# evoldoers/machineboss

Measured on NVIDIA B200. Metric: forward_viterbi_gcups, higher is better.
Workload: dtype f64

## Files before the change

machineboss_b200/csrc/mb_jit.cu:

```cuda
#include <cuda.h>
#include <dlfcn.h>
#include <nvrtc.h>
#include <unistd.h>

#include <algorithm>
#include <cmath>
#include <cstdio>
#include <cstring>
#include <map>
#include <mutex>
#include <sstream>

#include "mb_internal.h"
#include "mb_jit_skeleton.h"

namespace mb {

struct Driver {
  CUresult (*ModuleLoadData) (CUmodule*, const void*) = nullptr;
  CUresult (*ModuleUnload) (CUmodule) = nullptr;
  CUresult (*ModuleGetFunction) (CUfunction*, CUmodule, const char*) = nullptr;
  CUresult (*ModuleGetGlobal) (CUdeviceptr*, size_t*, CUmodule, const char*) = nullptr;
  CUresult (*LaunchKernel) (CUfunction, unsigned, unsigned, unsigned, unsigned, unsigned, unsigned, unsigned, CUstream, void**, void**) = nullptr;
  CUresult (*FuncSetAttribute) (CUfunction, CUfunction_attribute, int) = nullptr;
// ... 893 lines not shown
    o << "#ifndef MB_LDS\n"
         "template<int OFF> __device__ __forceinline__ double mb_lds (const unsigned addr) { double v; asm (\"ld.shared.f64 %0, [%1+%2];\" : \"=d\"(v) : \"r\"(addr), \"n\"(OFF)); return v; }\n"
         "#define MB_LDS(addr, off) mb_lds<off> (addr)\n#endif\n";
    o << "#define MB_PKW " << (passC * J.tbBytes + 3) / 4 << "      // 32-bit words of packed back-pointers per lane and step\n";
    o << "#ifndef MB_HOST_HARNESS\n"
         "// n = max (n, t) with the reference's tie-break (a later candidate wins only if strictly greater); with PTR the\n"
         "// winner's field value replaces the field in `word`: (word & ~field) | val, or a plain OR for a one-bit field\n"
         "template<bool PTR> __device__ __forceinline__ void mb_vmax (double& n, const double t, unsigned& word, const unsigned field, const unsigned val) {\n"
         "  if (!PTR) { if (n < t) n = t; return; }\n"
         "  if (field == val) asm (\"{ .reg .pred p; setp.lt.f64 p, %0, %2; selp.f64 %0, %2, %0, p; @p or.b32 %1, %1, %3; }\" : \"+d\"(n), \"+r\"(word) : \"d\"(t), \"r\"(val));\n"
         "  else asm (\"{ .reg .pred p; setp.lt.f64 p, %0, %2; selp.f64 %0, %2, %0, p; @p lop3.b32 %1, %1, %3, %4, 0xEA; }\" : \"+d\"(n), \"+r\"(word) : \"d\"(t), \"r\"(~field), \"r\"(val));\n"
         "}\n#endif\n\n";
    gen_cell_row_vit (o, m, J.fwd, J);
    gen_cell_row_lin (o, m, J.fwd, true);
    gen_cell_row_lin (o, m, J.bwd, false);
    o << "// MB_ROWCELLS_END\n";
  }
  gen_cell (o, m, J.fwd, true, false, J);
  gen_cell (o, m, J.bwd, false, false, J);
  gen_cell (o, m, J.fwd, true, true, J);
  gen_cell_counts (o, m, J);
  gen_cell_lin (o, m, J.fwd, true);
  gen_cell_lin (o, m, J.bwd, false);
  gen_cell_counts_lin (o, m, J);
  gen_fstore_lin (o, m, J);
  o << kJitSkeleton;
  return o.str();
}

int jit_host_tables (const mb_machine* m, int which, std::vector<double>& out) {
  std::string why;
  if (!jit_supported (m, &why)) { set_error ("machine not eligible for the JIT engine: " + why); return 1; }
  JitEngine J;
  generate (m, J);
  std::vector<double> ef, eb;
  fill_weights (m, J, ef, eb);
  RowTables f, b;
  row_tables (m, J.fwd, true, f);
  row_tables (m, J.bwd, false, b);
  const int nf = std::max (J.fwd.nSil, 1), nb = std::max (J.bwd.nSil, 1);
  out.clear();
  if (which == 0) out = f.rowLog;
  else if (which == 1) out = f.rowLinN;
  else if (which == 2) out = b.rowLinN;
  else if (which == 3) { const double* sp = (const double*) J.silParam.data(); out.assign (sp, sp + nf + nb); }
  else if (which == 4) {
    out.insert (out.end(), f.silN.begin(), f.silN.begin() + nf);
    out.insert (out.end(), b.silN.begin(), b.silN.begin() + nb);
    out.push_back (f.originInv); out.push_back (b.originInv); out.push_back (f.resLog); out.push_back (b.resLog);
  } else if (which == 5) out.push_back (f.ok && b.ok && J.linearOK ? 1. : 0.);
  else { set_error ("mb_jit_host_tables: which must be 0..5"); return 1; }
  return 0;
}

int jit_compile_check (const mb_machine* m, std::string* log) {
  std::string why;
  if (!jit_supported (m, &why)) { set_error ("machine not eligible for the JIT engine: " + why); return 1; }
  JitEngine J;
  generate (m, J);
  std::vector<char> cubin;
  if (nvrtc_compile (J.source, "", cubin, log)) return 1;
  if (!J.sourceV.empty()) {
    std::string logV;
    if (nvrtc_compile (J.sourceV, ".viterbi.cu", cubin, &logV)) return 1;
    if (log) *log += "\n---- Viterbi module (MB_C = " + std::to_string (J.CV) + ") ----\n" + logV;
  }
  if (m->opt.get ("jit_split", -1) > 0) {
    std::string logS;
    if (nvrtc_compile (J.sourceS, ".split.cu", cubin, &logS)) return 1;
    if (log) *log += "\n---- split-mode module ----\n" + logS;
  }
  return 0;
}

int jit_prepare (mb_machine* m) {
  JitEngine* Jp = new JitEngine;
  m->jit = Jp;
  JitEngine& J = *Jp;
  generate (m, J);
  if (compile (m, J)) return 1;

  std::vector<double> ef, eb;
  fill_weights (m, J, ef, eb);
  MB_CUDA (cudaMalloc (&J.dEmitF, ef.size() * 8));
  MB_CUDA (cudaMalloc (&J.dEmitB, eb.size() * 8));
  MB_CUDA (cudaMalloc (&J.dEmitFLin, ef.size() * 8));
  MB_CUDA (cudaMalloc (&J.dEmitBLin, eb.size() * 8));
  MB_CUDA (cudaMalloc (&J.dCounter, 8));
  if (jit_update_weights (m)) return 1;
  MB_CUDA (cudaMalloc (&J.dIdTabB, std::max<size_t> (J.bwd.idTab.size(), 1) * 4));
  MB_CUDA (cudaMemcpy (J.dIdTabB, J.bwd.idTab.data(), J.bwd.idTab.size() * 4, cudaMemcpyHostToDevice));
  std::vector<int32_t> plan;
  for (int v: J.fwd.stateSlot0) plan.push_back (v);
  for (auto& s: J.fwd.slots) plan.push_back (s.type);
  for (auto& s: J.fwd.slots) plan.push_back (s.other);
  for (auto& s: J.fwd.slots) plan.push_back (s.idOff);
  for (int v: J.shift) plan.push_back (v);
  for (int v: J.bits) plan.push_back (v);
  for (int v: J.fwd.idTab) plan.push_back (v);
  MB_CUDA (cudaMalloc (&J.dTbPlan, std::max<size_t> (plan.size(), 1) * 4));
  MB_CUDA (cudaMemcpy (J.dTbPlan, plan.data(), plan.size() * 4, cudaMemcpyHostToDevice));
  return 0;
}

void jit_destroy (mb_machine* m) {
  if (!m->jit) return;
  JitEngine* J = (JitEngine*) m->jit;
  if (J->mod && g_drv.ModuleUnload) g_drv.ModuleUnload (J->mod);
  if (J->modV && g_drv.ModuleUnload) g_drv.ModuleUnload (J->modV);
  if (J->modS && g_drv.ModuleUnload) g_drv.ModuleUnload (J->modS);
  for (auto& f: J->fit) if (f.mod && g_drv.ModuleUnload) g_drv.ModuleUnload (f.mod);
  if (J->dEmitF) cudaFree (J->dEmitF);
  if (J->dEmitB) cudaFree (J->dEmitB);
  if (J->dEmitFLin) cudaFree (J->dEmitFLin);
  if (J->dEmitBLin) cudaFree (J->dEmitBLin);
  if (J->dTbPlan) cudaFree (J->dTbPlan);
  if (J->dIdTabB) cudaFree (J->dIdTabB);
  if (J->dCounter) cudaFree (J->dCounter);
  if (J->dRowVit) cudaFree (J->dRowVit);
  if (J->dRowFLinN) cudaFree (J->dRowFLinN);
  if (J->dRowBLinN) cudaFree (J->dRowBLinN);
  delete J;
  m->jit = nullptr;
}

struct MBArgsHost {
  const uint8_t* x; const int64_t* xOff;
  const uint8_t* y; const int64_t* yOff;
  const int64_t* order; int64_t nWork; unsigned long long* counter;
  double* bnd; int64_t bndStride;
  double* result;
  const double* emit;
  uint8_t* tb; const int64_t* tbOff;
  double* F; const int64_t* fOff;
  const double* ll;
  double* counts;
  const int32_t* idTabB;
  int32_t* flag;
  unsigned* F32; const int64_t* f32Off;
  int32_t* ef; const int64_t* efOff;
  const int64_t* items; const int64_t* itemBnd; int* prog;
};

struct DevBuf {
  void* p = nullptr;
  ~DevBuf() { if (p) cudaFree (p); }
  int alloc (size_t bytes) { MB_CUDA (cudaMalloc (&p, bytes ? bytes : 8)); return 0; }
  template<class T> T* as() { return (T*) p; }
};

static std::vector<int64_t> cost_order (const mb_batch* b, const std::vector<int64_t>& pairs) {
  std::vector<int64_t> o = pairs;
  std::stable_sort (o.begin(), o.end(), [&] (int64_t p, int64_t q) {
    const double cp = (double) (b->xOff[p + 1] - b->xOff[p] + 1) * (double) (b->yOff[p + 1] - b->yOff[p] + 1);
    const double cq = (double) (b->xOff[q + 1] - b->xOff[q] + 1) * (double) (b->yOff[q + 1] - b->yOff[q] + 1);
    return cp > cq;
  });
  return o;
}

static const std::vector<int64_t>& full_order (mb_batch* b) {
  if ((int64_t) b->fullOrder.size() != b->nPairs) {
    std::vector<int64_t> all ((size_t) b->nPairs);
    for (int64_t k = 0; k < b->nPairs; ++k) all[k] = k;
    b->fullOrder = cost_order (b, all);
    b->wsOrderHoldsFull = false;
  }
  return b->fullOrder;
}

struct CountArgs { double* F = nullptr; const int64_t* fOff = nullptr; const double* ll = nullptr; double* counts = nullptr; int32_t* flag = nullptr;
                   unsigned* F32 = nullptr; const int64_t* f32Off = nullptr; int32_t* ef = nullptr; const int64_t* efOff = nullptr; };

static int launch (mb_machine* m, mb_batch* b, int which, const std::vector<int64_t>& order, double* dResult, uint8_t* dTb, const int64_t* dTbOff,
                   const CountArgs& ca = CountArgs(), int useC = 0) {
  JitEngine& J = *(JitEngine*) m->jit;
  const bool scoreKernel = which == 2 || which == 5 || which == 6 || which == 9;
  bool narrow = useC == J.C && useC != J.CV;
  const int scoreIdx = which == 2 ? 0 : which == 5 ? 1 : which == 6 ? 2 : 3;
  const JitEngine::FitModule* fitM = nullptr;
  if (scoreKernel && useC && useC != J.C && useC != J.CV) {
    for (auto& f: J.fit) if (f.C == useC) fitM = &f;
    if (!fitM) { set_error ("jit engine: no module fitted to " + std::to_string (useC) + " columns per lane"); return 1; }
  }
  if ((which == 5 || which == 6) && !J.normOK) { set_error ("jit engine: the normalised linear sweep was asked for a machine whose unit weights cannot be divided out"); return 1; }
  narrow = narrow && J.modV && scoreKernel;
  const bool rowTab = scoreKernel;
  const int slot = which;
  CUfunction fn = narrow ? (which == 2 ? J.kViterbiN : which == 5 ? J.kForwardLinN : which == 6 ? J.kBackwardLinN : J.kViterbiScoreN)
    : which == 9 ? J.kViterbiScore : which == 0 ? J.kForward : which == 1 ? J.kBackward : which == 2 ? J.kViterbi : which == 3 ? J.kFStore : which == 4 ? J.kBCounts : which == 5 ? J.kForwardLin : which == 6 ? J.kBackwardLin : which == 7 ? J.kFStoreLin : J.kBCountsLin;
  const bool lin = which >= 5 && which <= 8;
  int64_t maxLo = 0;
  for (int64_t k: order) maxLo = std::max (maxLo, b->yOff[k + 1] - b->yOff[k]);
  const int warpsPerBlock = J.threads / 32;
  int64_t grid = (int64_t) J.numSMs * (fitM ? fitM->blocksPerSM[scoreIdx] : narrow ? J.blocksPerSMN[scoreIdx] : J.blocksPerSM[slot]);
  if (fitM) fn = fitM->k[scoreIdx];
  const int W = 32 * (scoreKernel && J.modV ? J.CV : J.C);
  bool split = false;
  std::vector<int64_t> items, itemBnd;
  if (scoreKernel && !narrow && !fitM && m->opt.get ("jit_split", -1) != 0) {
    int64_t nItems = 0;
    for (int64_t k: order) nItems += (b->xOff[k + 1] - b->xOff[k] + W) / W;
    split = nItems > (int64_t) order.size() && (m->opt.get ("jit_split", -1) > 0 || (double) order.size() < 0.75 * (double) (grid * warpsPerBlock));
    if (split) {
      int64_t at = 0;
      for (int64_t k: order) {
        const int64_t nStrips = (b->xOff[k + 1] - b->xOff[k] + W) / W, Lo = b->yOff[k + 1] - b->yOff[k];
        if (nStrips > 0xffff) { split = false; break; }
        for (int64_t st = 0; st < nStrips; ++st) { items.push_back ((k << 16) | st); itemBnd.push_back (at); at += (Lo + 1) * (m->S + 1); }
      }
      itemBnd.push_back (at);
    }
  }
  if (split) {
    if (ensure_split_module (m, J)) return 1;
    const int q = which == 2 ? 0 : which == 5 ? 1 : which == 6 ? 2 : 3;
    fn = J.kSplit[q];
    grid = (int64_t) J.numSMs * J.blocksPerSMS[q];
  }
  const int64_t nWorkItems = split ? (int64_t) items.size() : (int64_t) order.size();
  grid = std::min<int64_t> (grid, (nWorkItems + warpsPerBlock - 1) / warpsPerBlock);
  grid = std::max<int64_t> (grid, 1);
  const int64_t bndStride = 2 * (maxLo + 1) * (m->S + 1);
  if (ws_bytes (b, WS_ORDER) < order.size() * 8) b->wsOrderHoldsFull = false;
  int64_t* dOrder = (int64_t*) ws_reserve (b, WS_ORDER, order.size() * 8);
  double* dBnd = (double*) ws_reserve (b, WS_BND, (size_t) (split ? itemBnd.back() + bndStride : grid * warpsPerBlock * bndStride) * 8);
  unsigned long long* dCounter = (unsigned long long*) ws_reserve (b, WS_COUNTER, 8);
  if (!dOrder || !dBnd || !dCounter) return 1;
  const bool isFull = &order == &b->fullOrder;
  if (!(isFull && b->wsOrderHoldsFull))
    MB_CUDA (cudaMemcpyAsync (dOrder, order.data(), order.size() * 8, cudaMemcpyHostToDevice, b->stream));
  b->wsOrderHoldsFull = isFull;
  MB_CUDA (cudaMemsetAsync (dCounter, 0, 8, b->stream));
  MBArgsHost A;
  A.x = b->dX; A.xOff = b->dXOff; A.y = b->dY; A.yOff = b->dYOff;
  A.order = dOrder; A.nWork = nWorkItems; A.counter = dCounter;
  A.items = nullptr; A.itemBnd = nullptr; A.prog = nullptr;
  if (split) {
    int64_t* dItems = (int64_t*) ws_reserve (b, WS_ITEMS, items.size() * 8);
    int64_t* dItemBnd = (int64_t*) ws_reserve (b, WS_ITEMBND, itemBnd.size() * 8);
    int* dProg = (int*) ws_reserve (b, WS_PROG, items.size() * 4);
    if (!dItems || !dItemBnd || !dProg) return 1;
    MB_CUDA (cudaMemcpyAsync (dItems, items.data(), items.size() * 8, cudaMemcpyHostToDevice, b->stream));
    MB_CUDA (cudaMemcpyAsync (dItemBnd, itemBnd.data(), itemBnd.size() * 8, cudaMemcpyHostToDevice, b->stream));
    MB_CUDA (cudaMemsetAsync (dProg, 0, items.size() * 4, b->stream));
    if (ca.flag) MB_CUDA (cudaMemsetAsync (ca.flag, 0, (size_t) b->nPairs * 4, b->stream));
    A.items = dItems; A.itemBnd = dItemBnd; A.prog = dProg;
  }
  A.bnd = dBnd; A.bndStride = bndStride;
  A.result = dResult;
  A.emit = (which == 5 || which == 7) ? J.dEmitFLin : (which == 6 || which == 8) ? J.dEmitBLin : (which == 1 || which == 4) ? J.dEmitB : J.dEmitF;
  if (rowTab) A.emit = which == 5 ? J.dRowFLinN : which == 6 ? J.dRowBLinN : J.dRowVit;
  A.flag = ca.flag;
  A.F32 = ca.F32; A.f32Off = ca.f32Off; A.ef = ca.ef; A.efOff = ca.efOff;
  A.tb = dTb; A.tbOff = dTbOff;
  A.F = ca.F; A.fOff = ca.fOff; A.ll = ca.ll; A.counts = ca.counts; A.idTabB = J.dIdTabB;
  if (m->opt.get ("verbose", 0))
    fprintf (stderr, "[mb_jit] kernel %d%s grid %lld x %d threads, %zu B smem, %d CTAs/SM, C=%d, %zu pairs, bnd %.1f MB\n", which, split ? " (split: strips as work items)" : rowTab && lin ? " (normalised)" : "", (long long) grid, J.threads,
             J.smemBytes[which], J.blocksPerSM[slot], fitM ? fitM->C : ((which == 2 || which == 5 || which == 6 || which == 9) && !narrow) ? J.CV : J.C, order.size(), (double) (grid * warpsPerBlock * bndStride) * 8 / 1e6);
  void* params[2] = { (rowTab && lin) ? (void*) J.silParamLinN.data() : lin ? (void*) J.silParamLin.data() : (void*) J.silParam.data(), (void*) &A };
  if (!cu_ok (g_drv.LaunchKernel (fn, (unsigned) grid, 1, 1, (unsigned) J.threads, 1, 1, (unsigned) J.smemBytes[which], (CUstream) b->stream, params, nullptr), "cuLaunchKernel")) return 1;
  return 0;
}

int jit_forward (mb_machine* m, mb_batch* b, double* loglike, bool backward) {
  JitEngine& J = *(JitEngine*) m->jit;
  if (b->nPairs == 0) return 0;
  const std::vector<int64_t>& order = full_order (b);
  double* dRes = (double*) ws_reserve (b, WS_RESULT, (size_t) b->nPairs * 8);
  if (!dRes) return 1;
  if (timing_begin (b)) return 1;
  int64_t launches = 1;
  if (J.linearOK && J.normOK) {
    int32_t* dFlag = (int32_t*) ws_reserve (b, WS_FLAG, (size_t) b->nPairs * 4);
    if (!dFlag) return 1;
    CountArgs ca;
    ca.flag = dFlag;
    if (launch (m, b, backward ? 6 : 5, order, dRes, nullptr, nullptr, ca, choose_width (m, J, b, order, 0))) return 1;
    std::vector<int32_t> flag ((size_t) b->nPairs);
    MB_CUDA (cudaMemcpyAsync (loglike, dRes, (size_t) b->nPairs * 8, cudaMemcpyDeviceToHost, b->stream));
    MB_CUDA (cudaMemcpyAsync (flag.data(), dFlag, (size_t) b->nPairs * 4, cudaMemcpyDeviceToHost, b->stream));
    MB_CUDA (cudaStreamSynchronize (b->stream));
    std::vector<int64_t> redo;
    for (int64_t k = 0; k < b->nPairs; ++k) if (flag[k] || !(loglike[k] > -INFINITY)) redo.push_back (k);
    b->lastRedo = (int64_t) redo.size();
    if (m->opt.get ("verbose", 0) && !redo.empty()) {
      int64_t nf[8] = { 0, 0, 0, 0, 0, 0, 0, 0 };
      for (int64_t k = 0; k < b->nPairs; ++k) ++nf[flag[k] & 7];
      fprintf (stderr, "[mb_jit] linear sweep flagged %lld of %lld pairs; by reason mask (1 spread, 2 neighbour frame, 4 boundary frame) 0..7: %lld %lld %lld %lld %lld %lld %lld %lld\n",
               (long long) redo.size(), (long long) b->nPairs, (long long) nf[0], (long long) nf[1], (long long) nf[2], (long long) nf[3], (long long) nf[4], (long long) nf[5], (long long) nf[6], (long long) nf[7]);
    }
    if (!redo.empty()) {
      if (launch (m, b, backward ? 1 : 0, cost_order (b, redo), dRes, nullptr, nullptr)) return 1;
      ++launches;
    }
  } else { b->lastRedo = 0; if (launch (m, b, backward ? 1 : 0, order, dRes, nullptr, nullptr)) return 1; }
  if (timing_end (b, launches)) return 1;
  MB_CUDA (cudaMemcpy (loglike, dRes, (size_t) b->nPairs * 8, cudaMemcpyDeviceToHost));
  return 0;
}

#define TB_MAXS 64
#define TB_MAXSLOTS 256
__global__ void __launch_bounds__(64) jit_traceback_kernel (TbPlan p, int nSlots, DevBatch b, const int64_t* __restrict__ pairs, int64_t nPairsHere,
                                      const uint8_t* __restrict__ tb, const int64_t* __restrict__ tbOff,
                                      const double* __restrict__ score, int64_t* __restrict__ len,
                                      uint8_t* __restrict__ tmp, const int64_t* __restrict__ tmpOff) {
  __shared__ unsigned perState[TB_MAXS + 1];
  __shared__ unsigned char slotMove[TB_MAXSLOTS], slotOther[TB_MAXSLOTS];
  for (int q = threadIdx.x; q <= p.S; q += blockDim.x)
    perState[q] = (q < p.S ? (unsigned) p.shift[q] | ((unsigned) p.bits[q] << 8) : 0u) | ((unsigned) p.stateSlot0[q] << 16);
  for (int q = threadIdx.x; q < nSlots; q += blockDim.x) {
    const int type = p.slotType[q];
    slotMove[q] = (unsigned char) (((type == T_MATCH || type == T_DELETE) ? 1 : 0) | ((type == T_MATCH || type == T_INSERT) ? 2 : 0));
    slotOther[q] = (unsigned char) p.slotOther[q];
  }
  __syncthreads();
  const int64_t slot = (int64_t) blockIdx.x * blockDim.x + threadIdx.x;
  if (slot >= nPairsHere) return;
  const int64_t k = pairs[slot];
  const int64_t Li = b.xOff[k + 1] - b.xOff[k], Lo = b.yOff[k + 1] - b.yOff[k];
  const uint8_t* base = tb + tbOff[k];
  uint8_t* out = tmp + tmpOff[slot + 1];
  int64_t n = 0;
  if (score[k] > -INFINITY) {
    int64_t i = Li, o = Lo;
    int s = p.S - 1;
    auto fetch = [&] (int64_t ii, int64_t oo) {
      const unsigned ui = (unsigned) ii, strip = ui / (unsigned) p.W, within = ui - strip * (unsigned) p.W, lane = within / (unsigned) p.C;
      const uint8_t* wp = base + ((((int64_t) strip * (Lo + 32) + oo + lane) * 32 + lane) * p.laneBytes + (within - lane * (unsigned) p.C) * p.tbBytes);
      if (within >= 8 && oo >= 8) asm volatile ("prefetch.global.L2 [%0];" :: "l"(wp - ((int64_t) (8 + 8 / p.C) * 32 + 8 / p.C) * p.laneBytes));
      unsigned long long w = 0;
      for (int q = 0; q < p.tbBytes; ++q) w |= (unsigned long long) wp[q] << (8 * q);
      return w;
    };
    unsigned long long word = fetch (i, o);
    while (i > 0 || o > 0 || s != 0) {
      const unsigned ps = perState[s];
      const int ptr = (int) ((word >> (ps & 0xffu)) & ((1ull << ((ps >> 8) & 0xffu)) - 1ull));
      const unsigned sl = (ps >> 16) + (unsigned) ptr;
      if (sl >= (perState[s + 1] >> 16)) break;
      ++n;
      out[-n] = (uint8_t) sl;
      const unsigned mv = slotMove[sl];
      s = slotOther[sl];
      if (mv) {
        i -= mv & 1u; o -= mv >> 1;
        if (i < 0 || o < 0) break;
        word = fetch (i, o);
      }
    }
  }
  len[slot] = n;
}

__global__ void __launch_bounds__(256) jit_path_ids_kernel (TbPlan p, int nSlots, DevBatch b, const int64_t* __restrict__ pairs, int64_t nPairsHere,
                                     const int64_t* __restrict__ len, const uint8_t* __restrict__ tmp, const int64_t* __restrict__ tmpOff,
                                     int32_t* __restrict__ out, const int64_t* __restrict__ outOff) {
  __shared__ int slotIdOff[TB_MAXSLOTS];
  __shared__ unsigned char slotType[TB_MAXSLOTS];
  for (int q = threadIdx.x; q < nSlots; q += blockDim.x) { slotIdOff[q] = p.slotIdOff[q]; slotType[q] = (unsigned char) p.slotType[q]; }
  __syncthreads();
  const int64_t slot = ((int64_t) blockIdx.x * blockDim.x + threadIdx.x) >> 5;
  const int lane = threadIdx.x & 31;
  if (slot >= nPairsHere) return;
  const int64_t k = pairs[slot];
  const uint8_t* x = b.x + b.xOff[k];
  const uint8_t* y = b.y + b.yOff[k];
  const int64_t n = len[slot];
  const uint8_t* src = tmp + tmpOff[slot + 1] - n;
  int32_t* dst = out + outOff[slot];
  int ci = 0, co = 0;
  for (int64_t q0 = 0; q0 < n; q0 += 32) {
    const int64_t q = q0 + lane;
    const int g = q < n ? src[q] : 0;
    const int type = q < n ? slotType[g] : T_SILENT;
    int mv = ((type == T_MATCH || type == T_DELETE) ? 1 : 0) | ((type == T_MATCH || type == T_INSERT) ? 0x10000 : 0);
#pragma unroll
    for (int d = 1; d < 32; d <<= 1) { const int up = __shfl_up_sync (0xffffffffu, mv, d); if (lane >= d) mv += up; }
    const int i = ci + (mv & 0xffff), o = co + (mv >> 16);
    if (q < n) {
      const int a = i ? x[i - 1] - 1 : 0, c = o ? y[o - 1] - 1 : 0;
      const int li = type == T_MATCH ? a * p.nOut + c : type == T_DELETE ? a : type == T_INSERT ? c : 0;
      dst[q] = p.idTab[slotIdOff[g] + li];
    }
    const int tot = __shfl_sync (0xffffffffu, mv, 31);
    ci += tot & 0xffff; co += tot >> 16;
  }
}


static size_t device_total_bytes (int device) {
  static size_t cache[64] = { 0 };
  if (device >= 0 && device < 64 && cache[device]) return cache[device];
  size_t freeB = 0, totalB = 0;
  if (cudaMemGetInfo (&freeB, &totalB) != cudaSuccess) return (size_t) 64 << 30;
  if (device >= 0 && device < 64) cache[device] = totalB;
  return totalB;
}

static double memory_budget (const mb_machine* m, const mb_batch* b, int slot, double wanted, const char* capOption) {
  const double cap = m->opt.has (capOption) ? (double) m->opt.get (capOption, 0) * 1048576.0 : 1e300;
  if (wanted <= (double) ws_bytes (b, slot)) return std::min (cap, (double) ws_bytes (b, slot));
  if (wanted <= cap && ws_pool_fits (b->device, (size_t) wanted)) return wanted;
  size_t freeB = 0, totalB = 0;
  if (cudaMemGetInfo (&freeB, &totalB) != cudaSuccess) return 0;
  return std::min (cap, std::min (0.85 * (double) (freeB + ws_bytes (b, slot) + ws_pool_bytes (b->device)), 0.5 * (double) totalB));
}

#define kKeepScratchBytes ((size_t) (0.6 * (double) device_total_bytes (b->device)))

int jit_viterbi (mb_machine* m, mb_batch* b, double* score, int64_t* pathLen) {
  JitEngine& J = *(JitEngine*) m->jit;
  b->pathStart.clear();
  b->pathLen.clear();
  if (b->nPairs == 0) return 0;
  const bool trace = pathLen != nullptr;
  const int useC = choose_width (m, J, b, full_order (b), trace ? 1 : 2);
  if (!trace) {
    double* dRes = (double*) ws_reserve (b, WS_RESULT2, (size_t) b->nPairs * 8);
    if (!dRes) return 1;
    if (timing_begin (b)) return 1;
    if (launch (m, b, 9, full_order (b), dRes, nullptr, nullptr, CountArgs(), useC)) return 1;
    if (timing_end (b, 1)) return 1;
    MB_CUDA (cudaMemcpy (score, dRes, (size_t) b->nPairs * 8, cudaMemcpyDeviceToHost));
    return 0;
  }
  const int W = 32 * useC;
  const int laneBytes = useC * J.tbBytes;
  const bool padded = laneBytes != 1 && laneBytes != 2 && laneBytes != 4 && laneBytes != 8 && laneBytes != 16;
  const int64_t stepBytes = 32 * (padded ? 16 : laneBytes);
  double wanted = 0;
  for (int64_t k = 0; k < b->nPairs; ++k)
    wanted += (double) (((((b->xOff[k + 1] - b->xOff[k]) + W) / W) * ((b->yOff[k + 1] - b->yOff[k]) + 32) * stepBytes + 255) & ~(int64_t) 255);
  const double budget = memory_budget (m, b, WS_TB, wanted, "jit_tb_budget_mb");
  std::vector<std::vector<int64_t>> chunks (1);
  std::vector<int64_t> tbOffHost ((size_t) b->nPairs, 0);
  std::vector<int64_t> chunkBytes (1, 0);
  for (int64_t k = 0; k < b->nPairs; ++k) {
    const int64_t Li = b->xOff[k + 1] - b->xOff[k], Lo = b->yOff[k + 1] - b->yOff[k];
    int64_t need = ((Li + W) / W) * (Lo + 32) * stepBytes;
    need = (need + 255) & ~(int64_t) 255;
    if ((double) need > budget) { set_error ("pair " + std::to_string (k) + ": Viterbi back-pointers do not fit in device memory"); return 1; }
    if (!chunks.back().empty() && (double) (chunkBytes.back() + need) > budget) { chunks.emplace_back(); chunkBytes.push_back (0); }
    tbOffHost[k] = chunkBytes.back();
    chunkBytes.back() += need;
    chunks.back().push_back (k);
  }
  int64_t maxChunk = 0;
  for (int64_t v: chunkBytes) maxChunk = std::max (maxChunk, v);
  uint8_t* dTb = (uint8_t*) ws_reserve (b, WS_TB, (size_t) maxChunk);
  double* dRes = (double*) ws_reserve (b, WS_RESULT2, (size_t) b->nPairs * 8);
  int64_t* dTbOff = (int64_t*) ws_reserve (b, WS_TBOFF, (size_t) b->nPairs * 8);
  int64_t* dPairs = (int64_t*) ws_reserve (b, WS_PAIRS, (size_t) b->nPairs * 8);
  int64_t* dLen = (int64_t*) ws_reserve (b, WS_LEN, (size_t) b->nPairs * 8);
  int64_t* dOutOff = (int64_t*) ws_reserve (b, WS_OUTOFF, (size_t) b->nPairs * 8);
  if (!dTb || !dRes || !dTbOff || !dPairs || !dLen || !dOutOff) return 1;
  MB_CUDA (cudaMemcpyAsync (dTbOff, tbOffHost.data(), (size_t) b->nPairs * 8, cudaMemcpyHostToDevice, b->stream));
  if (trace) { b->pathStart.assign ((size_t) b->nPairs, 0); b->pathLen.assign ((size_t) b->nPairs, 0); }
  char* plan = (char*) J.dTbPlan;
  const size_t nSlots = J.fwd.slots.size();
  TbPlan tp;
  tp.stateSlot0 = (const int32_t*) plan;
  tp.slotType = tp.stateSlot0 + (m->S + 1);
  tp.slotOther = tp.slotType + nSlots;
  tp.slotIdOff = tp.slotOther + nSlots;
  tp.shift = tp.slotIdOff + nSlots;
  tp.bits = tp.shift + m->S;
  tp.idTab = tp.bits + m->S;
  tp.S = m->S; tp.nOut = m->nOut; tp.tbBytes = J.tbBytes; tp.W = W;
  tp.C = useC; tp.laneBytes = padded ? 16 : laneBytes;
  int64_t packed = 0, launches = 0;
  double ms = 0;
  for (size_t c = 0; c < chunks.size(); ++c) {
    std::vector<int64_t> chunkOrder;
    if (chunks.size() > 1) chunkOrder = cost_order (b, chunks[c]);
    const std::vector<int64_t>& order = chunks.size() > 1 ? chunkOrder : full_order (b);
    if (timing_begin (b)) return 1;
    if (launch (m, b, 2, order, dRes, dTb, dTbOff, CountArgs(), useC)) return 1;
    ++launches;
    if (trace) {
      const size_t n = chunks[c].size();
      const int64_t depth = (int64_t) m->fwdLevelOff.size() - 1;
      std::vector<int64_t> tmpOff (n + 1, 0);
      for (size_t q = 0; q < n; ++q) {
        const int64_t k = chunks[c][q];
        tmpOff[q + 1] = tmpOff[q] + ((b->xOff[k + 1] - b->xOff[k]) + (b->yOff[k + 1] - b->yOff[k]) + 1) * depth;
      }
      uint8_t* dTmp = (uint8_t*) ws_reserve (b, WS_PATHTMP, (size_t) tmpOff[n]);
      int64_t* dTmpOff = (int64_t*) ws_reserve (b, WS_PATHTMPOFF, (n + 1) * 8);
      if (!dTmp || !dTmpOff) return 1;
      MB_CUDA (cudaMemcpyAsync (dPairs, chunks[c].data(), n * 8, cudaMemcpyHostToDevice, b->stream));
      MB_CUDA (cudaMemcpyAsync (dTmpOff, tmpOff.data(), (n + 1) * 8, cudaMemcpyHostToDevice, b->stream));
      const unsigned tg = (unsigned) ((n + 63) / 64);
      jit_traceback_kernel<<<tg, 64, 0, b->stream>>> (tp, (int) nSlots, b->dev, dPairs, (int64_t) n, dTb, dTbOff, dRes, dLen, dTmp, dTmpOff);
      MB_CUDA (cudaGetLastError());
      std::vector<int64_t> len (n), off (n);
      MB_CUDA (cudaMemcpyAsync (len.data(), dLen, n * 8, cudaMemcpyDeviceToHost, b->stream));
      MB_CUDA (cudaStreamSynchronize (b->stream));
      for (size_t q = 0; q < n; ++q) {
        off[q] = packed;
        b->pathStart[chunks[c][q]] = packed;
        b->pathLen[chunks[c][q]] = len[q];
        packed += len[q];
      }
      if (paths_reserve (b, packed)) return 1;
      MB_CUDA (cudaMemcpyAsync (dOutOff, off.data(), n * 8, cudaMemcpyHostToDevice, b->stream));
      jit_path_ids_kernel<<<(unsigned) ((n * 32 + 255) / 256), 256, 0, b->stream>>> (tp, (int) nSlots, b->dev, dPairs, (int64_t) n, dLen, dTmp, dTmpOff, b->dPaths, dOutOff);
      MB_CUDA (cudaGetLastError());
      launches += 2;
    }
    if (timing_end (b, launches)) return 1;
    ms += b->lastMs;
  }
  b->lastMs = ms;
  b->lastLaunches = launches;
  MB_CUDA (cudaMemcpy (score, dRes, (size_t) b->nPairs * 8, cudaMemcpyDeviceToHost));
  if (trace) for (int64_t k = 0; k < b->nPairs; ++k) pathLen[k] = b->pathLen[k];
  if (ws_bytes (b, WS_TB) > kKeepScratchBytes) ws_release (b, WS_TB);
  return 0;
}

static int counts_log (mb_machine* m, mb_batch* b, const std::vector<int64_t>& pairs, bool wantCounts,
                       std::vector<double>& hostCounts, double* loglike, int64_t& launches, double& ms) {
  if (pairs.empty()) return 0;
  double wanted = 0;
  for (int64_t k: pairs) wanted += 8.0 * (double) (((((b->xOff[k + 1] - b->xOff[k]) + 1) * ((b->yOff[k + 1] - b->yOff[k]) + 1) * m->S) + 31) & ~(int64_t) 31);
  const double budget = memory_budget (m, b, WS_F, wanted, "jit_f_budget_mb") / 8.0;
  std::vector<std::vector<int64_t>> chunks (1);
  std::vector<int64_t> fOffHost ((size_t) b->nPairs, 0), chunkDoubles (1, 0);
  for (int64_t k: pairs) {
    const int64_t Li = b->xOff[k + 1] - b->xOff[k], Lo = b->yOff[k + 1] - b->yOff[k];
    const int64_t need = (((Li + 1) * (Lo + 1) * m->S) + 31) & ~(int64_t) 31;
    if ((double) need > budget) { set_error ("pair " + std::to_string (k) + ": the Forward matrix does not fit in device memory"); return 1; }
    if (!chunks.back().empty() && (double) (chunkDoubles.back() + need) > budget) { chunks.emplace_back(); chunkDoubles.push_back (0); }
    fOffHost[k] = chunkDoubles.back();
    chunkDoubles.back() += need;
    chunks.back().push_back (k);
  }
  int64_t maxChunk = 0;
  for (int64_t v: chunkDoubles) maxChunk = std::max (maxChunk, v);
  const size_t T = (size_t) std::max<int64_t> (m->T, 1);
  double* dF = (double*) ws_reserve (b, WS_F, (size_t) maxChunk * 8);
  double* dLL = (double*) ws_reserve (b, WS_RESULT, (size_t) b->nPairs * 8);
  double* dBack = (double*) ws_reserve (b, WS_RESULT2, (size_t) b->nPairs * 8);
  int64_t* dFOff = (int64_t*) ws_reserve (b, WS_FOFF, (size_t) b->nPairs * 8);
  double* dCounts = (double*) ws_reserve (b, WS_COUNTS, T * 8);
  if (!dF || !dLL || !dBack || !dFOff || !dCounts) return 1;
  MB_CUDA (cudaMemcpyAsync (dFOff, fOffHost.data(), (size_t) b->nPairs * 8, cudaMemcpyHostToDevice, b->stream));
  MB_CUDA (cudaMemsetAsync (dCounts, 0, T * 8, b->stream));
  for (size_t c = 0; c < chunks.size(); ++c) {
    const std::vector<int64_t> order = cost_order (b, chunks[c]);
    CountArgs ca;
    ca.F = dF; ca.fOff = dFOff; ca.ll = dLL; ca.counts = dCounts;
    if (timing_begin (b)) return 1;
    if (launch (m, b, 3, order, dLL, nullptr, nullptr, ca)) return 1;
    ++launches;
    if (wantCounts) { if (launch (m, b, 4, order, dBack, nullptr, nullptr, ca)) return 1; ++launches; }
    if (timing_end (b, launches)) return 1;
    ms += b->lastMs;
  }
  std::vector<double> ll ((size_t) b->nPairs), cnt (T);
  MB_CUDA (cudaMemcpy (ll.data(), dLL, (size_t) b->nPairs * 8, cudaMemcpyDeviceToHost));
  for (int64_t k: pairs) loglike[k] = ll[k];
  if (wantCounts) {
    MB_CUDA (cudaMemcpy (cnt.data(), dCounts, T * 8, cudaMemcpyDeviceToHost));
    for (int64_t t = 0; t < m->T; ++t) hostCounts[t] += cnt[t];
  }
  if (ws_bytes (b, WS_F) > kKeepScratchBytes) ws_release (b, WS_F);
  return 0;
}

static int counts_lin (mb_machine* m, mb_batch* b, const std::vector<int64_t>& pairs, bool wantCounts,
                       std::vector<double>& hostCounts, double* loglike, int64_t& launches, double& ms) {
  JitEngine& J = *(JitEngine*) m->jit;
  const int W = 32 * J.C;
  double wanted = 0;
  for (int64_t k: pairs)
    wanted += 4.0 * (double) ((((b->xOff[k + 1] - b->xOff[k]) + W) / W) * ((b->yOff[k + 1] - b->yOff[k]) + 32) * (int64_t) (32 * J.C * J.storeQ * 4));
  const double budget = memory_budget (m, b, WS_F, wanted, "jit_f_budget_mb") / 4.0;
  std::vector<std::vector<int64_t>> chunks (1);
  std::vector<int64_t> fOffHost ((size_t) b->nPairs, 0), efOffHost ((size_t) b->nPairs, 0), chunkWords (1, 0), chunkEf (1, 0);
  for (int64_t k: pairs) {
    const int64_t Li = b->xOff[k + 1] - b->xOff[k], Lo = b->yOff[k + 1] - b->yOff[k];
    const int64_t need = ((Li + W) / W) * (Lo + 32) * (int64_t) (32 * J.C * J.storeQ * 4);
    const int64_t needEf = ((Li + W) / W) * ((Lo + 32 + 15) / 16);
    if ((double) need > budget) { set_error ("pair " + std::to_string (k) + ": the Forward matrix does not fit in device memory"); return 1; }
    if (!chunks.back().empty() && (double) (chunkWords.back() + need) > budget) { chunks.emplace_back(); chunkWords.push_back (0); chunkEf.push_back (0); }
    fOffHost[k] = chunkWords.back();
    efOffHost[k] = chunkEf.back();
    chunkWords.back() += need;
    chunkEf.back() += needEf;
    chunks.back().push_back (k);
  }
  int64_t maxChunk = 0, maxEf = 0;
  for (int64_t v: chunkWords) maxChunk = std::max (maxChunk, v);
  for (int64_t v: chunkEf) maxEf = std::max (maxEf, v);
  const size_t T = (size_t) std::max<int64_t> (m->T, 1);
  unsigned* dF32 = (unsigned*) ws_reserve (b, WS_F, (size_t) maxChunk * 4);
  int32_t* dEf = (int32_t*) ws_reserve (b, WS_EF, (size_t) std::max<int64_t> (maxEf, 1) * 4);
  double* dLL = (double*) ws_reserve (b, WS_RESULT, (size_t) b->nPairs * 8);
  double* dBack = (double*) ws_reserve (b, WS_RESULT2, (size_t) b->nPairs * 8);
  int64_t* dFOff = (int64_t*) ws_reserve (b, WS_FOFF, (size_t) b->nPairs * 8);
  int64_t* dEfOff = (int64_t*) ws_reserve (b, WS_EFOFF, (size_t) b->nPairs * 8);
  double* dCounts = (double*) ws_reserve (b, WS_COUNTS, T * 8);
  int32_t* dFlag = (int32_t*) ws_reserve (b, WS_FLAG, (size_t) b->nPairs * 4);
  if (!dF32 || !dEf || !dLL || !dBack || !dFOff || !dEfOff || !dCounts || !dFlag) return 1;
  MB_CUDA (cudaMemcpyAsync (dFOff, fOffHost.data(), (size_t) b->nPairs * 8, cudaMemcpyHostToDevice, b->stream));
  MB_CUDA (cudaMemcpyAsync (dEfOff, efOffHost.data(), (size_t) b->nPairs * 8, cudaMemcpyHostToDevice, b->stream));
  std::vector<int64_t> redo;
  std::vector<double> ll ((size_t) b->nPairs), cnt (T);
  std::vector<int32_t> flag ((size_t) b->nPairs);
  for (size_t c = 0; c < chunks.size(); ++c) {
    CountArgs ca;
    ca.F32 = dF32; ca.f32Off = dFOff; ca.ef = dEf; ca.efOff = dEfOff; ca.ll = dLL; ca.counts = dCounts; ca.flag = dFlag;
    if (timing_begin (b)) return 1;
    MB_CUDA (cudaMemsetAsync (dFlag, 0, (size_t) b->nPairs * 4, b->stream));
    if (launch (m, b, 7, cost_order (b, chunks[c]), dLL, nullptr, nullptr, ca)) return 1;
    ++launches;
    MB_CUDA (cudaMemcpyAsync (ll.data(), dLL, (size_t) b->nPairs * 8, cudaMemcpyDeviceToHost, b->stream));
    MB_CUDA (cudaMemcpyAsync (flag.data(), dFlag, (size_t) b->nPairs * 4, cudaMemcpyDeviceToHost, b->stream));
    MB_CUDA (cudaStreamSynchronize (b->stream));
    std::vector<int64_t> good;
    for (int64_t k: chunks[c]) {
      if (flag[k] || !(ll[k] > -INFINITY)) redo.push_back (k);
      else { good.push_back (k); loglike[k] = ll[k]; }
    }
    if (wantCounts && !good.empty()) {
      MB_CUDA (cudaMemsetAsync (dCounts, 0, T * 8, b->stream));
      MB_CUDA (cudaMemsetAsync (dFlag, 0, (size_t) b->nPairs * 4, b->stream));
      if (launch (m, b, 8, cost_order (b, good), dBack, nullptr, nullptr, ca)) return 1;
      ++launches;
      MB_CUDA (cudaMemcpyAsync (flag.data(), dFlag, (size_t) b->nPairs * 4, cudaMemcpyDeviceToHost, b->stream));
      MB_CUDA (cudaMemcpyAsync (cnt.data(), dCounts, T * 8, cudaMemcpyDeviceToHost, b->stream));
      MB_CUDA (cudaStreamSynchronize (b->stream));
      bool anyFlag = false;
      for (int64_t k: good) anyFlag |= flag[k] != 0;
      if (anyFlag) redo.insert (redo.end(), good.begin(), good.end());
      else for (int64_t t = 0; t < m->T; ++t) hostCounts[t] += cnt[t];
    }
    if (timing_end (b, launches)) return 1;
    ms += b->lastMs;
  }
  if (ws_bytes (b, WS_F) > kKeepScratchBytes) ws_release (b, WS_F);
  b->lastRedo = (int64_t) redo.size();
  std::sort (redo.begin(), redo.end());
  return counts_log (m, b, redo, wantCounts, hostCounts, loglike, launches, ms);
}

int jit_counts (mb_machine* m, mb_batch* b, double* counts, double* loglike) {
  JitEngine& J = *(JitEngine*) m->jit;
  if (counts) for (int64_t t = 0; t < m->T; ++t) counts[t] = 0;
  if (b->nPairs == 0) return 0;
  std::vector<int64_t> all ((size_t) b->nPairs);
  for (int64_t k = 0; k < b->nPairs; ++k) all[k] = k;
  std::vector<double> hostCounts ((size_t) std::max<int64_t> (m->T, 1), 0.), ll ((size_t) b->nPairs, 0.);
  int64_t launches = 0;
  double ms = 0;
  const int rc = J.linearOK ? counts_lin (m, b, all, counts != nullptr, hostCounts, ll.data(), launches, ms)
                            : counts_log (m, b, all, counts != nullptr, hostCounts, ll.data(), launches, ms);
  if (rc) return rc;
  b->lastMs = ms;
  b->lastLaunches = launches;
  if (loglike) for (int64_t k = 0; k < b->nPairs; ++k) loglike[k] = ll[k];
  if (counts) for (int64_t t = 0; t < m->T; ++t) counts[t] = hostCounts[t];
  return 0;
}

}
```

Measured before the change: 7018.

## Stage Viterbi traceback through shared-memory windows and compute path offsets on device

The traceback kernel now gives each pair to a warp instead of a thread. The warp streams the pair's back-pointer strip into a double-buffered shared-memory window with cp.async and prefetches the next window into L2, while lane 0 walks the path. The last block to finish computes path output offsets with an on-device prefix sum. Chunks become contiguous pair ranges, which removes the host round-trip (length copy, stream sync, offset upload) between the traceback and path-id kernels. The cost is serial single-lane walking inside each warp and extra shared memory. It also adds an atomic last-block pattern whose counter must be reset correctly across chunks.

```diff
diff --git a/machineboss_b200/csrc/mb_jit.cu b/machineboss_b200/csrc/mb_jit.cu
--- a/machineboss_b200/csrc/mb_jit.cu
+++ b/machineboss_b200/csrc/mb_jit.cu
@@ -1219,60 +1219,126 @@
 
 #define TB_MAXS 64
 #define TB_MAXSLOTS 256
-__global__ void __launch_bounds__(64) jit_traceback_kernel (TbPlan p, int nSlots, DevBatch b, const int64_t* __restrict__ pairs, int64_t nPairsHere,
+#define TB_THREADS 128
+static const int kTbWindowBytes = 2048;
+__global__ void __launch_bounds__(TB_THREADS) jit_traceback_kernel (TbPlan p, int nSlots, DevBatch b, int64_t k0, int64_t nPairsHere,
                                       const uint8_t* __restrict__ tb, const int64_t* __restrict__ tbOff,
                                       const double* __restrict__ score, int64_t* __restrict__ len,
-                                      uint8_t* __restrict__ tmp, const int64_t* __restrict__ tmpOff) {
+                                      uint8_t* __restrict__ tmp, const int64_t* __restrict__ tmpEnd,
+                                      int64_t* __restrict__ outOff, int64_t* __restrict__ total, unsigned* __restrict__ blocksDone, int first) {
   __shared__ unsigned perState[TB_MAXS + 1];
-  __shared__ unsigned char slotMove[TB_MAXSLOTS], slotOther[TB_MAXSLOTS];
+  __shared__ unsigned char slotGroup[TB_MAXSLOTS];
+  __shared__ __align__(16) uint8_t win[TB_THREADS / 32][2][kTbWindowBytes];
+  __shared__ int64_t segSum[TB_THREADS];
+  __shared__ bool last;
   for (int q = threadIdx.x; q <= p.S; q += blockDim.x)
     perState[q] = (q < p.S ? (unsigned) p.shift[q] | ((unsigned) p.bits[q] << 8) : 0u) | ((unsigned) p.stateSlot0[q] << 16);
   for (int q = threadIdx.x; q < nSlots; q += blockDim.x) {
     const int type = p.slotType[q];
-    slotMove[q] = (unsigned char) (((type == T_MATCH || type == T_DELETE) ? 1 : 0) | ((type == T_MATCH || type == T_INSERT) ? 2 : 0));
-    slotOther[q] = (unsigned char) p.slotOther[q];
+    slotGroup[q] = (unsigned char) (((type == T_MATCH || type == T_DELETE) ? 1 : 0) | ((type == T_MATCH || type == T_INSERT) ? 2 : 0) | (p.slotOther[q] << 2));
   }
   __syncthreads();
-  const int64_t slot = (int64_t) blockIdx.x * blockDim.x + threadIdx.x;
-  if (slot >= nPairsHere) return;
-  const int64_t k = pairs[slot];
-  const int64_t Li = b.xOff[k + 1] - b.xOff[k], Lo = b.yOff[k + 1] - b.yOff[k];
-  const uint8_t* base = tb + tbOff[k];
-  uint8_t* out = tmp + tmpOff[slot + 1];
-  int64_t n = 0;
-  if (score[k] > -INFINITY) {
-    int64_t i = Li, o = Lo;
-    int s = p.S - 1;
-    auto fetch = [&] (int64_t ii, int64_t oo) {
-      const unsigned ui = (unsigned) ii, strip = ui / (unsigned) p.W, within = ui - strip * (unsigned) p.W, lane = within / (unsigned) p.C;
-      const uint8_t* wp = base + ((((int64_t) strip * (Lo + 32) + oo + lane) * 32 + lane) * p.laneBytes + (within - lane * (unsigned) p.C) * p.tbBytes);
-      if (within >= 8 && oo >= 8) asm volatile ("prefetch.global.L2 [%0];" :: "l"(wp - ((int64_t) (8 + 8 / p.C) * 32 + 8 / p.C) * p.laneBytes));
-      unsigned long long w = 0;
-      for (int q = 0; q < p.tbBytes; ++q) w |= (unsigned long long) wp[q] << (8 * q);
-      return w;
-    };
-    unsigned long long word = fetch (i, o);
-    while (i > 0 || o > 0 || s != 0) {
-      const unsigned ps = perState[s];
-      const int ptr = (int) ((word >> (ps & 0xffu)) & ((1ull << ((ps >> 8) & 0xffu)) - 1ull));
-      const unsigned sl = (ps >> 16) + (unsigned) ptr;
-      if (sl >= (perState[s + 1] >> 16)) break;
-      ++n;
-      out[-n] = (uint8_t) sl;
-      const unsigned mv = slotMove[sl];
-      s = slotOther[sl];
-      if (mv) {
-        i -= mv & 1u; o -= mv >> 1;
-        if (i < 0 || o < 0) break;
-        word = fetch (i, o);
+  const int lane = threadIdx.x & 31, warp = threadIdx.x >> 5;
+  const unsigned W = (unsigned) p.W, C = (unsigned) p.C;
+  const int stepBytes = 32 * p.laneBytes, winSteps = kTbWindowBytes / stepBytes;
+  for (int64_t q = (int64_t) blockIdx.x * (TB_THREADS / 32) + warp; q < nPairsHere; q += (int64_t) gridDim.x * (TB_THREADS / 32)) {
+    const int64_t k = k0 + q;
+    const int Li = (int) (b.xOff[k + 1] - b.xOff[k]), Lo = (int) (b.yOff[k + 1] - b.yOff[k]);
+    const uint8_t* base = tb + tbOff[k];
+    uint8_t* out = tmp + tmpEnd[k];
+    int n = 0;
+    if (score[k] > -INFINITY) {
+      int i = Li, o = Lo, s = p.S - 1, done = 0;
+      int strip = (int) ((unsigned) Li / W), t = o + (int) (((unsigned) Li - (unsigned) strip * W) / C);
+      int wi = t / winSteps, cur = 0;
+      auto fetch = [&] (const int buf, const int st, const int w, const bool ahead) {
+        const int s0 = w * winSteps, s1 = min (s0 + winSteps, Lo + 32);
+        const uint8_t* src = base + ((int64_t) st * (Lo + 32) + s0) * stepBytes;
+        for (int c = lane; c < (s1 - s0) * stepBytes / 16; c += 32)
+          asm volatile ("cp.async.cg.shared.global [%0], [%1], 16;" :: "r"((unsigned) __cvta_generic_to_shared (&win[warp][buf][16 * c])), "l"(src + 16 * c));
+        asm volatile ("cp.async.commit_group;");
+        if (ahead && w > 0 && lane * 128 < kTbWindowBytes)
+          asm volatile ("prefetch.global.L2 [%0];" :: "l"(src - (int64_t) winSteps * stepBytes + lane * 128));
+      };
+      fetch (cur, strip, wi, false);
+      for (;;) {
+        if (wi > 0) fetch (cur ^ 1, strip, wi - 1, true);
+        else asm volatile ("cp.async.commit_group;");
+        asm volatile ("cp.async.wait_group 1;" ::: "memory");
+        __syncwarp();
+        int at = strip;
+        if (lane == 0) {
+          const uint8_t* wb = &win[warp][cur][0];
+          for (;;) {
+            const unsigned within = (unsigned) i - (unsigned) strip * W, ln = within / C;
+            const uint8_t* wp = wb + (t - wi * winSteps) * stepBytes + ln * p.laneBytes + (within - ln * C) * p.tbBytes;
+            unsigned long long word = 0;
+            for (int c = 0; c < p.tbBytes; ++c) word |= (unsigned long long) wp[c] << (8 * c);
+            unsigned mv = 0;
+            while (!mv) {
+              if (i == 0 && o == 0 && s == 0) { done = 1; break; }
+              const unsigned ps = perState[s];
+              const unsigned sl = (ps >> 16) + (unsigned) ((word >> (ps & 0xffu)) & ((1ull << ((ps >> 8) & 0xffu)) - 1ull));
+              if (sl >= (perState[s + 1] >> 16)) { done = 1; break; }
+              out[-(++n)] = (uint8_t) sl;
+              const unsigned g = slotGroup[sl];
+              s = (int) (g >> 2);
+              mv = g & 3u;
+            }
+            if (done) break;
+            i -= (int) (mv & 1u); o -= (int) (mv >> 1);
+            if (i < 0 || o < 0) { done = 1; break; }
+            at = (int) ((unsigned) i / W);
+            t = o + (int) (((unsigned) i - (unsigned) at * W) / C);
+            if (at != strip || t < wi * winSteps) break;
+          }
+        }
+        i = __shfl_sync (0xffffffffu, i, 0); o = __shfl_sync (0xffffffffu, o, 0); s = __shfl_sync (0xffffffffu, s, 0);
+        n = __shfl_sync (0xffffffffu, n, 0); done = __shfl_sync (0xffffffffu, done, 0);
+        const int st = __shfl_sync (0xffffffffu, at, 0);
+        t = __shfl_sync (0xffffffffu, t, 0);
+        __syncwarp();
+        if (done) break;
+        const int w = t / winSteps;
+        if (st == strip && w == wi - 1) { cur ^= 1; wi = w; }
+        else {
+          asm volatile ("cp.async.wait_group 0;" ::: "memory");
+          __syncwarp();
+          strip = st; wi = w;
+          fetch (cur, strip, wi, false);
+        }
       }
-    }
-  }
-  len[slot] = n;
-}
-
-__global__ void __launch_bounds__(256) jit_path_ids_kernel (TbPlan p, int nSlots, DevBatch b, const int64_t* __restrict__ pairs, int64_t nPairsHere,
-                                     const int64_t* __restrict__ len, const uint8_t* __restrict__ tmp, const int64_t* __restrict__ tmpOff,
+      asm volatile ("cp.async.wait_group 0;" ::: "memory");
+      __syncwarp();
+    }
+    if (lane == 0) len[k] = n;
+  }
+  __syncthreads();
+  if (threadIdx.x == 0) {
+    __threadfence();
+    last = atomicAdd (blocksDone, 1u) == gridDim.x - 1;
+  }
+  __syncthreads();
+  if (!last) return;
+  __threadfence();
+  const int64_t per = (nPairsHere + TB_THREADS - 1) / TB_THREADS, q0 = min (nPairsHere, per * threadIdx.x), q1 = min (nPairsHere, q0 + per);
+  int64_t sum = 0;
+  for (int64_t q = q0; q < q1; ++q) sum += __ldcg (len + k0 + q);
+  segSum[threadIdx.x] = sum;
+  __syncthreads();
+  if (threadIdx.x == 0) {
+    int64_t run = first ? 0 : *total;
+    for (int q = 0; q < TB_THREADS; ++q) { const int64_t v = segSum[q]; segSum[q] = run; run += v; }
+    *total = run;
+    *blocksDone = 0;
+  }
+  __syncthreads();
+  int64_t run = segSum[threadIdx.x];
+  for (int64_t q = q0; q < q1; ++q) { outOff[k0 + q] = run; run += __ldcg (len + k0 + q); }
+}
+
+__global__ void __launch_bounds__(256) jit_path_ids_kernel (TbPlan p, int nSlots, DevBatch b, int64_t k0, int64_t nPairsHere,
+                                     const int64_t* __restrict__ len, const uint8_t* __restrict__ tmp, const int64_t* __restrict__ tmpEnd,
                                      int32_t* __restrict__ out, const int64_t* __restrict__ outOff) {
   __shared__ int slotIdOff[TB_MAXSLOTS];
   __shared__ unsigned char slotType[TB_MAXSLOTS];
@@ -1281,12 +1347,12 @@
   const int64_t slot = ((int64_t) blockIdx.x * blockDim.x + threadIdx.x) >> 5;
   const int lane = threadIdx.x & 31;
   if (slot >= nPairsHere) return;
-  const int64_t k = pairs[slot];
+  const int64_t k = k0 + slot;
   const uint8_t* x = b.x + b.xOff[k];
   const uint8_t* y = b.y + b.yOff[k];
-  const int64_t n = len[slot];
-  const uint8_t* src = tmp + tmpOff[slot + 1] - n;
-  int32_t* dst = out + outOff[slot];
+  const int64_t n = len[k];
+  const uint8_t* src = tmp + tmpEnd[k] - n;
+  int32_t* dst = out + outOff[k];
   int ci = 0, co = 0;
   for (int64_t q0 = 0; q0 < n; q0 += 32) {
     const int64_t q = q0 + lane;
@@ -1351,30 +1417,36 @@
   for (int64_t k = 0; k < b->nPairs; ++k)
     wanted += (double) (((((b->xOff[k + 1] - b->xOff[k]) + W) / W) * ((b->yOff[k + 1] - b->yOff[k]) + 32) * stepBytes + 255) & ~(int64_t) 255);
   const double budget = memory_budget (m, b, WS_TB, wanted, "jit_tb_budget_mb");
-  std::vector<std::vector<int64_t>> chunks (1);
-  std::vector<int64_t> tbOffHost ((size_t) b->nPairs, 0);
-  std::vector<int64_t> chunkBytes (1, 0);
+  const int64_t depth = (int64_t) m->fwdLevelOff.size() - 1;
+  std::vector<int64_t> chunkFirst (1, 0), chunkBytes (1, 0), chunkPath (1, 0);
+  std::vector<int64_t> tbOffHost ((size_t) b->nPairs, 0), pathEndHost ((size_t) b->nPairs, 0);
+  int64_t maxPathSlots = 0;
   for (int64_t k = 0; k < b->nPairs; ++k) {
     const int64_t Li = b->xOff[k + 1] - b->xOff[k], Lo = b->yOff[k + 1] - b->yOff[k];
     int64_t need = ((Li + W) / W) * (Lo + 32) * stepBytes;
     need = (need + 255) & ~(int64_t) 255;
     if ((double) need > budget) { set_error ("pair " + std::to_string (k) + ": Viterbi back-pointers do not fit in device memory"); return 1; }
-    if (!chunks.back().empty() && (double) (chunkBytes.back() + need) > budget) { chunks.emplace_back(); chunkBytes.push_back (0); }
+    if (k > chunkFirst.back() && (double) (chunkBytes.back() + need) > budget) { chunkFirst.push_back (k); chunkBytes.push_back (0); chunkPath.push_back (0); }
     tbOffHost[k] = chunkBytes.back();
     chunkBytes.back() += need;
-    chunks.back().push_back (k);
-  }
-  int64_t maxChunk = 0;
-  for (int64_t v: chunkBytes) maxChunk = std::max (maxChunk, v);
+    chunkPath.back() += (Li + Lo + 1) * depth;
+    pathEndHost[k] = chunkPath.back();
+    maxPathSlots += (Li + Lo + 1) * depth;
+  }
+  chunkFirst.push_back (b->nPairs);
+  int64_t maxChunk = 0, maxChunkPath = 0;
+  for (size_t c = 0; c + 1 < chunkFirst.size(); ++c) { maxChunk = std::max (maxChunk, chunkBytes[c]); maxChunkPath = std::max (maxChunkPath, chunkPath[c]); }
+  if (paths_reserve (b, maxPathSlots)) return 1;
   uint8_t* dTb = (uint8_t*) ws_reserve (b, WS_TB, (size_t) maxChunk);
   double* dRes = (double*) ws_reserve (b, WS_RESULT2, (size_t) b->nPairs * 8);
   int64_t* dTbOff = (int64_t*) ws_reserve (b, WS_TBOFF, (size_t) b->nPairs * 8);
-  int64_t* dPairs = (int64_t*) ws_reserve (b, WS_PAIRS, (size_t) b->nPairs * 8);
   int64_t* dLen = (int64_t*) ws_reserve (b, WS_LEN, (size_t) b->nPairs * 8);
-  int64_t* dOutOff = (int64_t*) ws_reserve (b, WS_OUTOFF, (size_t) b->nPairs * 8);
-  if (!dTb || !dRes || !dTbOff || !dPairs || !dLen || !dOutOff) return 1;
+  int64_t* dOutOff = (int64_t*) ws_reserve (b, WS_OUTOFF, (size_t) b->nPairs * 8 + 16);
+  uint8_t* dTmp = (uint8_t*) ws_reserve (b, WS_PATHTMP, (size_t) maxChunkPath);
+  int64_t* dTmpEnd = (int64_t*) ws_reserve (b, WS_PATHTMPOFF, (size_t) b->nPairs * 8);
+  if (!dTb || !dRes || !dTbOff || !dLen || !dOutOff || !dTmp || !dTmpEnd) return 1;
   MB_CUDA (cudaMemcpyAsync (dTbOff, tbOffHost.data(), (size_t) b->nPairs * 8, cudaMemcpyHostToDevice, b->stream));
-  if (trace) { b->pathStart.assign ((size_t) b->nPairs, 0); b->pathLen.assign ((size_t) b->nPairs, 0); }
+  MB_CUDA (cudaMemcpyAsync (dTmpEnd, pathEndHost.data(), (size_t) b->nPairs * 8, cudaMemcpyHostToDevice, b->stream));
   char* plan = (char*) J.dTbPlan;
   const size_t nSlots = J.fwd.slots.size();
   TbPlan tp;
@@ -1387,53 +1459,41 @@
   tp.idTab = tp.bits + m->S;
   tp.S = m->S; tp.nOut = m->nOut; tp.tbBytes = J.tbBytes; tp.W = W;
   tp.C = useC; tp.laneBytes = padded ? 16 : laneBytes;
-  int64_t packed = 0, launches = 0;
-  double ms = 0;
-  for (size_t c = 0; c < chunks.size(); ++c) {
+  int64_t* dTotal = dOutOff + b->nPairs;
+  unsigned* dBlocksDone = (unsigned*) (dOutOff + b->nPairs + 1);
+  MB_CUDA (cudaMemsetAsync (dTotal, 0, 16, b->stream));
+  const size_t nChunks = chunkFirst.size() - 1;
+  int64_t launches = 0;
+  if (timing_begin (b)) return 1;
+  for (size_t c = 0; c < nChunks; ++c) {
+    const int64_t k0 = chunkFirst[c], n = chunkFirst[c + 1] - k0;
     std::vector<int64_t> chunkOrder;
-    if (chunks.size() > 1) chunkOrder = cost_order (b, chunks[c]);
-    const std::vector<int64_t>& order = chunks.size() > 1 ? chunkOrder : full_order (b);
-    if (timing_begin (b)) return 1;
+    if (nChunks > 1) {
+      std::vector<int64_t> pairs ((size_t) n);
+      for (int64_t q = 0; q < n; ++q) pairs[q] = k0 + q;
+      chunkOrder = cost_order (b, pairs);
+    }
+    const std::vector<int64_t>& order = nChunks > 1 ? chunkOrder : full_order (b);
     if (launch (m, b, 2, order, dRes, dTb, dTbOff, CountArgs(), useC)) return 1;
-    ++launches;
-    if (trace) {
-      const size_t n = chunks[c].size();
-      const int64_t depth = (int64_t) m->fwdLevelOff.size() - 1;
-      std::vector<int64_t> tmpOff (n + 1, 0);
-      for (size_t q = 0; q < n; ++q) {
-        const int64_t k = chunks[c][q];
-        tmpOff[q + 1] = tmpOff[q] + ((b->xOff[k + 1] - b->xOff[k]) + (b->yOff[k + 1] - b->yOff[k]) + 1) * depth;
-      }
-      uint8_t* dTmp = (uint8_t*) ws_reserve (b, WS_PATHTMP, (size_t) tmpOff[n]);
-      int64_t* dTmpOff = (int64_t*) ws_reserve (b, WS_PATHTMPOFF, (n + 1) * 8);
-      if (!dTmp || !dTmpOff) return 1;
-      MB_CUDA (cudaMemcpyAsync (dPairs, chunks[c].data(), n * 8, cudaMemcpyHostToDevice, b->stream));
-      MB_CUDA (cudaMemcpyAsync (dTmpOff, tmpOff.data(), (n + 1) * 8, cudaMemcpyHostToDevice, b->stream));
-      const unsigned tg = (unsigned) ((n + 63) / 64);
-      jit_traceback_kernel<<<tg, 64, 0, b->stream>>> (tp, (int) nSlots, b->dev, dPairs, (int64_t) n, dTb, dTbOff, dRes, dLen, dTmp, dTmpOff);
-      MB_CUDA (cudaGetLastError());
-      std::vector<int64_t> len (n), off (n);
-      MB_CUDA (cudaMemcpyAsync (len.data(), dLen, n * 8, cudaMemcpyDeviceToHost, b->stream));
-      MB_CUDA (cudaStreamSynchronize (b->stream));
-      for (size_t q = 0; q < n; ++q) {
-        off[q] = packed;
-        b->pathStart[chunks[c][q]] = packed;
-        b->pathLen[chunks[c][q]] = len[q];
-        packed += len[q];
-      }
-      if (paths_reserve (b, packed)) return 1;
-      MB_CUDA (cudaMemcpyAsync (dOutOff, off.data(), n * 8, cudaMemcpyHostToDevice, b->stream));
-      jit_path_ids_kernel<<<(unsigned) ((n * 32 + 255) / 256), 256, 0, b->stream>>> (tp, (int) nSlots, b->dev, dPairs, (int64_t) n, dLen, dTmp, dTmpOff, b->dPaths, dOutOff);
-      MB_CUDA (cudaGetLastError());
-      launches += 2;
-    }
-    if (timing_end (b, launches)) return 1;
-    ms += b->lastMs;
-  }
-  b->lastMs = ms;
-  b->lastLaunches = launches;
-  MB_CUDA (cudaMemcpy (score, dRes, (size_t) b->nPairs * 8, cudaMemcpyDeviceToHost));
-  if (trace) for (int64_t k = 0; k < b->nPairs; ++k) pathLen[k] = b->pathLen[k];
+    jit_traceback_kernel<<<(unsigned) ((n + TB_THREADS / 32 - 1) / (TB_THREADS / 32)), TB_THREADS, 0, b->stream>>> (tp, (int) nSlots, b->dev, k0, n, dTb, dTbOff, dRes, dLen,
+                                                                                                                  dTmp, dTmpEnd, dOutOff, dTotal, dBlocksDone, c == 0);
+    MB_CUDA (cudaGetLastError());
+    jit_path_ids_kernel<<<(unsigned) ((n * 32 + 255) / 256), 256, 0, b->stream>>> (tp, (int) nSlots, b->dev, k0, n, dLen, dTmp, dTmpEnd, b->dPaths, dOutOff);
+    MB_CUDA (cudaGetLastError());
+    launches += 3;
+  }
+  std::vector<int64_t> len ((size_t) b->nPairs);
+  MB_CUDA (cudaMemcpyAsync (score, dRes, (size_t) b->nPairs * 8, cudaMemcpyDeviceToHost, b->stream));
+  MB_CUDA (cudaMemcpyAsync (len.data(), dLen, (size_t) b->nPairs * 8, cudaMemcpyDeviceToHost, b->stream));
+  if (timing_end (b, launches)) return 1;
+  b->pathStart.assign ((size_t) b->nPairs, 0);
+  b->pathLen.assign ((size_t) b->nPairs, 0);
+  int64_t packed = 0;
+  for (int64_t k = 0; k < b->nPairs; ++k) {
+    b->pathStart[k] = packed;
+    b->pathLen[k] = pathLen[k] = len[k];
+    packed += len[k];
+  }
   if (ws_bytes (b, WS_TB) > kKeepScratchBytes) ws_release (b, WS_TB);
   return 0;
 }
```

After: 6297 (median of 6 runs). -10.3%, worse.
